# vvvwo/KSS-ICP

Measured on AMD Instinct MI355X. Metric: icp_iterations_per_sec, higher is better.
Workload: dtype f32; 1 GPU; C2: one 100000x100000 uniform-sphere pair per GPU, 50 fixed ICP iterations + fitness pass per step (exact NN + cov reduce + host 3x3 SVD), R_z(10deg), jitter 1e-3; n_src=100000, n_tgt=100000, pairs_per_gpu=1, nn_engine=cell list + brute-force fallback, nn_arithmetic=reference (no fma)

## Files before the change

### kss-icp_amd/csrc/kss_ctx.hpp

```cpp
#pragma once
#include <dlfcn.h>
#include <hip/hip_runtime.h>

#include <algorithm>
#include <atomic>
#include <chrono>
#include <cmath>
#include <cstdio>
#include <cstdlib>
#include <cstring>
#include <mutex>
#include <string>
#include <thread>
#include <vector>

#include "kss_internal.hpp"
#include "kss_host_pool.hpp"

using namespace kss;

struct DevBuf {
    void* p = nullptr;
    size_t cap = 0;
};
// ... 16 lines not shown
    double grid_stats[8] = {0, 0, 0, 0, 0, 0, 0, 0};
    double last_setup_ms = 0, last_loop_ms = 0;
    double t_launch_us = 0, t_wait_us = 0, t_host_us = 0;
    bool timing = false;
    bool tables_staged = false;
    int64_t stats_ns = -1, stats_nt = -1;

    DevBuf tgt4, src0, cur[2], keys, partials, sums, nn_work, red_work, pair_red, state, cs, scratch_a,
        scratch_b, scratch_c, stage_src, stage_tgt, stage_idx, stage_d2, stage_out, g_counts, g_slot, g_start, g_cursor,
        g_bsums, g_sorted, g_list, g_count, g_bbox, g_partials, g_start2, g_pairs, g_stamps, g_pos, g_nnst, res_pos, res_wc, res_perm, pack_seg, reg_s, reg_t, reg_p, reg_all, reg_f, reg_g, oct_pts, oct_cen, oct_a, oct_b, oct_tmp, pre_partials, pre_state, g_rowpair, g_gate;
    DevBuf p2l_idx, p2l_d2, p2l_perm, p2l_rows, p2l_nrm, p2l_n64;
    DevBuf trim_rows, trim_state;
    DevBuf rob_keys;
    DevBuf gicp_snrm;
    DevBuf pb_desc, pb_rowpair, pb_nrm;
    DevBuf pb_rscale;
    DevBuf pb_snrm, pb_gicp;
    DevBuf o2o_table, o2o_idx, o2o_d2;
    DevBuf recip_sorted, recip_box, recip_grids;
    std::vector<RecipPairDev> h_recip_grids;
    int64_t recip_total_cells = 0;
    void* h_gicp = nullptr; size_t h_gicp_cap = 0;
    void* h_gicp_dev = nullptr;
    const PairState* last_state_dev = nullptr;
    HostPool pool;
    std::vector<kss_vmap*> vmaps;
    std::vector<kss_ctx*> workers;
    std::vector<unsigned long long> last_stamps;
    int stamps_nblk = 0; unsigned long long stamps_seq = 0;
    std::vector<float> h_bbox;
    unsigned int* h_box = nullptr; unsigned int* h_box_dev = nullptr; size_t h_box_bytes = 0;
    unsigned box_tag = 0; int box_rows = 0;
    double evals_sum = 0.0, evals_launches = 0.0;
    void* h_sums = nullptr;  size_t h_sums_cap = 0;
    void* h_sums_dev = nullptr;
    void* h_p2l = nullptr; size_t h_p2l_cap = 0;
    void* h_p2l_dev = nullptr;
    unsigned long long* h_seq = nullptr;
    unsigned long long* h_seq_dev = nullptr;
    size_t h_seq_bytes = 0;
    struct Gated {
        int supported = -1;
        bool want_next = false;
        bool pending = false;
        bool chain = false;
        int steps_left = 0;
        int max_steps = 1;
        int slot = 0;
        unsigned long long seq = 0;
        int32_t stamp = 0;
        const void* d_in = nullptr; void* d_out = nullptr;
        bool fma = false, full = false, want_full = false; double max_d2 = 0.0;
    } gated;
    bool ws_dirty = false;
    bool defer_wait = false;
    PairState* h_xf = nullptr; PairState* h_xf_dev = nullptr;
    bool fit_last = false;
    bool nn_have = false;
    BarBuf gate_bar, res_gate, bar_state;
    int large_bar = -1;
    unsigned res_launches = 0;
    double res_passes = 0.0;
    int cand_cap = 0, cand_cap_pad = -1, cand_cap_fma = -1;
    int spec_judge = -1; double spec_threshold = 0.0; bool spec_ran = false, spec_cancelled = false;
    std::chrono::steady_clock::time_point res_backoff[2] = {};
    unsigned long long seq = 0;
    void* h_state = nullptr; size_t h_state_cap = 0;

    int prof = 0;
    unsigned prof_tick[KSS_K_COUNT] = {};
    struct EvPair { hipEvent_t a, b; };
    std::vector<EvPair> ev[KSS_K_COUNT];
    std::vector<EvPair> ev_pool;
    double prof_ms[KSS_K_COUNT] = {0};
    int64_t prof_n[KSS_K_COUNT] = {0};
};

static inline int set_err(kss_ctx* c, int code, const char* what, hipError_t e = hipSuccess) {
    if (c) {
        c->err = what;
        if (e != hipSuccess) { c->err += ": "; c->err += hipGetErrorString(e); }
    }
    return code;
}

#define HIPCHK(ctx, call)                                                        \
    do {                                                                         \
        hipError_t e_ = (call);                                                  \
        if (e_ != hipSuccess) return set_err((ctx), KSS_ERR_HIP, #call, e_);     \
    } while (0)

static inline int ensure(kss_ctx* c, DevBuf& b, size_t bytes) {
    if (bytes <= b.cap) return KSS_OK;
    if (b.p) {
        HIPCHK(c, hipStreamSynchronize(c->stream));
        HIPCHK(c, hipFree(b.p));
        b.p = nullptr; b.cap = 0;
    }
    size_t want = bytes + bytes / 8 + 256;
    hipError_t e = hipMalloc(&b.p, want);
    if (e != hipSuccess) { b.p = nullptr; return set_err(c, KSS_ERR_NOMEM, "hipMalloc", e); }
    b.cap = want;
    return KSS_OK;
}

static inline int ensure_zeroed(kss_ctx* c, DevBuf& b, size_t bytes) {
// ... 145 lines not shown
```

### kss-icp_amd/csrc/kss_engine.hip

```cpp
#pragma clang fp contract(off)

#include <emmintrin.h>
#include <limits>

#include "kss_ctx.hpp"
#include "kss_pair_device.hpp"

namespace kss {

static int restore_zero_at_rest(kss_ctx* c);

static int resident_rows_limit(kss_ctx* c) {
    if (c->cu_count <= 0) {
        hipDeviceProp_t prop;
        c->cu_count = hipGetDeviceProperties(&prop, c->device) == hipSuccess && prop.multiProcessorCount > 0 ? prop.multiProcessorCount : 1;
        (void)hipGetLastError();
    }
    return c->cu_count;
}

constexpr int PUB_PAIRS = 32;
static int ensure_pub(kss_ctx* c, int npairs = PUB_PAIRS);

struct PairGeom {
// ... 440 lines not shown
static void gated_cancel(kss_ctx* c);

static inline bool collect_pair(kss_ctx* c, int p, unsigned long long want) {
    const unsigned long long* sl = c->h_seq + (size_t)2 * NSUMS * p;
    double* out = (double*)c->h_sums + (size_t)NSUMS * p;
    if (!slots_collect(sl + 2 * (NSUMS - 1), 1, want, out + NSUMS - 1)) return false;
    return slots_collect(sl, NSUMS, want, out);
}

static int wait_pair(kss_ctx* c, int p, unsigned long long want) {
    for (long spin = 0; spin < 2000000; ++spin) {
        if (collect_pair(c, p, want)) return KSS_OK;
        __builtin_ia32_pause();
    }
    return KSS_ERR_HIP;
}

static int wait_seq(kss_ctx* c, int npairs = 1, unsigned long long want = 0, const int* active = nullptr, bool* not_published = nullptr) {
    if (!want) want = c->seq;
    bool slow = false;
    for (int p = npairs - 1; p >= 0; --p) {
        if (active && !active[p]) continue;
        if (!slow && wait_pair(c, p, want) == KSS_OK) continue;
        if (!slow) {
            gated_cancel(c);
            HIPCHK(c, hipStreamSynchronize(c->stream));
            slow = true;
        }
        if (!collect_pair(c, p, want)) {
            if (not_published) *not_published = true;
            return set_err(c, KSS_ERR_HIP, "kernel finished without publishing its result");
        }
    }
    return KSS_OK;
}

int ensure_pub_slots(kss_ctx* c) { return ensure_pub(c); }
int wait_slots(kss_ctx* c, int nslots, double* out) {
    const unsigned long long want = c->seq;
    for (long spin = 0; spin < 2000000; ++spin) {
        if (slots_collect(c->h_seq, nslots, want, out)) return KSS_OK;
        __builtin_ia32_pause();
    }
    HIPCHK(c, hipStreamSynchronize(c->stream));
    if (!slots_collect(c->h_seq, nslots, want, out)) return set_err(c, KSS_ERR_HIP, "kernel finished without publishing its result");
    return KSS_OK;
}

static bool gated_available(kss_ctx* c) {
    static const bool want = getenv("KSS_GATED") == nullptr || atoi(getenv("KSS_GATED")) != 0;
    if (!want || !c->own_stream || kss_live_contexts().load() != 1) return false;
    if (c->gated.supported < 0) {
        c->gated.supported = 0;
        if (bar_ensure(c, c->gate_bar, 256)) {
            c->gated.supported = 1;
            return true;
        }
        void *x = nullptr, *xd = nullptr;
        if (ensure(c, c->g_gate, 256) == KSS_OK && hipMemsetAsync(c->g_gate.p, 0, 256, c->stream) == hipSuccess &&
            hipHostMalloc(&x, 2 * sizeof(PairState), hipHostMallocMapped) == hipSuccess && hipHostGetDevicePointer(&xd, x, 0) == hipSuccess) {
            std::memset(x, 0, 2 * sizeof(PairState));
            c->h_xf = (PairState*)x; c->h_xf_dev = (PairState*)xd;
            c->gated.supported = 1;
        } else {
            (void)hipGetLastError();
            if (x) hipHostFree(x);
        }
    }
    return c->gated.supported == 1;
}

static void gated_release(kss_ctx* c, const PairState& st, int skip) {
    if (c->gate_bar.p) {
        unsigned words[16];
        std::memcpy(words, &st, sizeof st);
        words[14] = (unsigned)skip;
        static const long torn_at = getenv("KSS_TEST_TORN_GATE") ? atol(getenv("KSS_TEST_TORN_GATE")) : -1;
        static long released = 0;
        gate_record_store((unsigned*)c->gate_bar.p + 32 * c->gated.slot, words, (unsigned)c->gated.stamp, ++released == torn_at);
    } else {
        PairState* rec = &c->h_xf[c->gated.slot];
        for (int k = 0; k < 12; ++k) rec->m[k] = st.m[k];
        rec->active = st.active; rec->apply = st.apply; rec->pad[0] = skip;
        __atomic_store_n(&rec->pad[1], c->gated.stamp, __ATOMIC_RELEASE);
    }
    kss_ctx::Gated& G = c->gated;
    if (!skip && --G.steps_left > 0) {
        G.slot ^= 1;
        G.stamp += 1;
        G.seq += 1;
        const void* in = G.d_out; G.d_out = const_cast<void*>(G.d_in); G.d_in = in;
    } else {
        G.pending = false;
        G.steps_left = 0;
    }
}

static void gated_cancel(kss_ctx* c) {
    if (!c->gated.pending) return;
    PairState none;
    std::memset(&none, 0, sizeof none);
    gated_release(c, none, 1);
}

struct GatedGuard {
    kss_ctx* c;
    explicit GatedGuard(kss_ctx* c_) : c(c_) {}
    ~GatedGuard() { gated_cancel(c); c->gated.want_next = false; }
};

static float skin_setting() {
    static const float skin = getenv("KSS_SKIN") ? (float)atof(getenv("KSS_SKIN")) : 0.25f;
    return skin;
}
static int gate_polls_setting() {
    static const int gate_polls = getenv("KSS_GATE_POLLS") ? atoi(getenv("KSS_GATE_POLLS")) : (1 << 22);
    return gate_polls;
}

static PassArgs pass_args(kss_ctx* c, const IcpPlan& pl, const float4* d_in, float4* d_out, double max_d2,
                          int32_t* d_idx_out, float* d_d2_out) {
    PassArgs a;
    std::memset(&a, 0, sizeof a);
    a.src_in = d_in; a.src_out = d_out;
    a.cell_start = (const int32_t*)c->g_start.p + 1;
    a.sorted = (const float4*)c->g_sorted.p;
    a.tgt4 = (const float4*)c->tgt4.p;
    a.nn_win = (float4*)c->g_pos.p;
    a.nn_state = (float2*)c->g_nnst.p;
    a.skin = skin_setting();
    a.chain_len = 1;
    a.gate_polls = gate_polls_setting();
    a.chained = d_in != (const float4*)c->src0.p ? 1 : c->fit_last ? 2 : 0;
    a.src_last0 = (const float4*)c->cur[0].p; a.src_last1 = (const float4*)c->cur[1].p;
    a.keys = (unsigned long long*)c->keys.p;
    a.list = (int32_t*)c->g_list.p; a.list_count = (int32_t*)c->g_count.p;
    a.total_rows = pl.total_rows;
    a.use_prev = c->nn_have ? 1 : 0;
    a.max_d2 = max_d2;
    a.rows = (Granule*)c->partials.p;
    a.pub = c->h_seq_dev;
    a.idx_out = d_idx_out; a.d2_out = d_d2_out;
    {
        static const long torn_at = getenv("KSS_TEST_TORN_SLOT") ? atol(getenv("KSS_TEST_TORN_SLOT")) : -1;
        static long launches = 0;
        a.test_torn = torn_at > 0 && ++launches == torn_at ? 1 : 0;
    }
    if (pl.gridb) {
        a.pairs = (const GridPairDev*)c->g_pairs.p;
        a.row_pair = (const int32_t*)c->g_rowpair.p;
        a.defer_pairs = pl.npairs > resident_rows_limit(c) ? pl.npairs : 0;
    } else {
        a.pair0 = pl.gpairs[0];
    }
    return a;
}

struct GridPass {
    const IcpPlan& pl;
    bool fma, full;
    const float4* d_in; float4* d_out;
    double max_d2;
    int32_t* d_idx_out; float* d_d2_out;
    PassArgs a;
    int nblk;
    unsigned long long* stamps2 = nullptr;
    bool plain_args = false;
    unsigned long long want_seq = 0;
    bool via_gate = false;
};

static void grid_launch_plain(kss_ctx* c, GridPass& g) {
    ProfScope ps(c, KSS_K_GRID_NN);
    g.a.ps0 = ((const PairState*)c->h_state)[0];
    g.a.seq = ++c->seq;
    if (g.stamps2) g.a.stamps = g.stamps2 + (size_t)(g.a.seq & 1) * g.nblk * 16;
    launch_grid_pass(c->stream, g.fma, g.full, false, true, g.a);
    c->nn_have = true;
    g.want_seq = c->seq;
}

static void grid_release_or_launch(kss_ctx* c, GridPass& g) {
    kss_ctx::Gated& G = c->gated;
    if (G.pending && G.d_in == (const void*)g.d_in && G.d_out == (void*)g.d_out && G.fma == g.fma && G.full == g.full && G.max_d2 == g.max_d2 && g.plain_args) {
        g.want_seq = G.seq;
        c->seq = std::max(c->seq, G.seq);
        if (G.chain && c->prof > 0) c->prof_n[KSS_K_GRID_CHAIN_PASS] += 1;
        g.via_gate = true;
        static const long drop_at = getenv("KSS_TEST_DROP_GATE") ? atol(getenv("KSS_TEST_DROP_GATE")) : -1;
        static long releases = 0;
        if (++releases == drop_at) { G.pending = false; G.steps_left = 0; }
        else gated_release(c, ((const PairState*)c->h_state)[0], 0);
    } else {
        gated_cancel(c);
        grid_launch_plain(c, g);
    }
}

static void grid_enqueue_next(kss_ctx* c, const GridPass& g) {
    kss_ctx::Gated& G = c->gated;
    const bool next_sampled = c->prof == 1 || (c->prof > 1 && c->prof_tick[KSS_K_GRID_NN] % (unsigned)c->prof == 0);
    static const bool want_chain = getenv("KSS_CHAIN") == nullptr || atoi(getenv("KSS_CHAIN")) != 0;
    int len = 1;
    if (G.want_next && !G.pending && g.plain_args && gated_available(c) && want_chain && c->gate_bar.p &&
        (g.pl.total_rows <= resident_rows_limit(c) || g.pl.total_rows == 1))
        len = std::max(1, std::min(G.max_steps, 1 << 16));
    if (!(G.want_next && !G.pending && g.plain_args && gated_available(c) && (len > 1 || !next_sampled))) return;
    if (c->prof > 1 && len == 1) ++c->prof_tick[KSS_K_GRID_NN];
    float4* nxt_out = g.d_out == (float4*)c->cur[0].p ? (float4*)c->cur[1].p : (float4*)c->cur[0].p;
    G.slot ^= 1;
    G.stamp = (G.stamp + 1) & 0x7fffffff;
    if (G.stamp == 0 || G.stamp > 0x7fffffff - len - 1) G.stamp = 1;
    PassArgs n = pass_args(c, g.pl, g.d_out, nxt_out, g.max_d2, nullptr, nullptr);
    n.ps0 = ((const PairState*)c->h_state)[0];
    n.gate_seq = G.stamp;
    if (c->gate_bar.p) {
        n.state = nullptr;
        n.gate_dev = (unsigned int*)c->gate_bar.p;
        n.gate_slot = G.slot;
        n.chain_len = len;
        n.src_alt = g.d_out;
    } else {
        n.state = c->h_xf_dev + G.slot;
        n.gate_dev = (unsigned int*)c->g_gate.p;
    }
    n.seq = c->seq + 1;
    if (g.stamps2) n.stamps = g.stamps2 + (size_t)(n.seq & 1) * g.nblk * 16;
    if (len > 1) {
        ProfScope ps(c, KSS_K_GRID_CHAIN, true);
        launch_grid_pass(c->stream, g.fma, G.want_full, false, true, n);
    } else {
        launch_grid_pass(c->stream, g.fma, G.want_full, false, true, n);
    }
    G.chain = len > 1;
    G.pending = true; G.steps_left = len; G.seq = n.seq; G.d_in = g.d_out; G.d_out = nxt_out; G.fma = g.fma; G.full = G.want_full; G.max_d2 = g.max_d2;
    if (hipGetLastError() != hipSuccess) { gated_cancel(c); G.supported = 0; }
}

static int grid_wait(kss_ctx* c, GridPass& g) {
    bool not_published = false;
    const int rcw = wait_seq(c, 1, g.want_seq, nullptr, &not_published);
    if (rcw == KSS_OK || !g.via_gate || !not_published) return rcw;
    c->gated.pending = false; c->gated.steps_left = 0;
    c->err.clear();
    std::fprintf(stderr, "[kss] a waiting kernel was not answered in time and left; the pass is launched again\n");
    c->ws_dirty = true;
    KCHK(restore_zero_at_rest(c));
    grid_launch_plain(c, g);
    HIPCHK(c, hipGetLastError());
    return wait_seq(c, 1, g.want_seq);
}

static int grid_stamps_arm(kss_ctx* c, GridPass& g) {
    static const int stamps_mode = getenv("KSS_GRID_STAMPS") ? atoi(getenv("KSS_GRID_STAMPS")) : 0;
    if (stamps_mode == 1) {
        KCHK(ensure(c, c->g_stamps, (size_t)g.nblk * 16 * sizeof(unsigned long long)));
        HIPCHK(c, hipMemsetAsync(c->g_stamps.p, 0, (size_t)g.nblk * 16 * sizeof(unsigned long long), c->stream));
        g.a.stamps = (unsigned long long*)c->g_stamps.p;
    } else if (stamps_mode == 2) {
        KCHK(ensure(c, c->g_stamps, (size_t)g.nblk * 32 * sizeof(unsigned long long)));
        g.stamps2 = (unsigned long long*)c->g_stamps.p;
        c->stamps_nblk = g.nblk;
    }
    return KSS_OK;
}
static int grid_stamps_read(kss_ctx* c, const GridPass& g) {
    if (g.stamps2) { c->stamps_seq = g.want_seq; return KSS_OK; }
    if (!g.a.stamps) return KSS_OK;
    c->last_stamps.resize((size_t)g.nblk * 16);
    HIPCHK(c, hipMemcpy(c->last_stamps.data(), g.a.stamps, c->last_stamps.size() * sizeof(unsigned long long), hipMemcpyDeviceToHost));
    for (int b = 0; b < g.nblk; ++b) c->evals_sum += (double)c->last_stamps[(size_t)b * 16 + 10];
    c->evals_launches += 1.0;
    return KSS_OK;
}

static int grid_list_fallback(kss_ctx* c, const GridPass& g) {
    const IcpPlan& pl = g.pl;
    gated_cancel(c);
    c->gated.want_next = false;
    KCHK(stage_tables(c, pl));
    {
        PairState one;
        std::memset(&one, 0, sizeof one);
        one.active = 1;
        HIPCHK(c, hipMemcpy(c->state.p, &one, sizeof one, hipMemcpyHostToDevice));
    }
    if (getenv("KSS_LIST_CHECK")) {
        HIPCHK(c, hipStreamSynchronize(c->stream));
// ... 200 lines not shown
static int pair_ninfo(const PairMode& M) { return M.sim ? KSS_SIM_NINFO : M.mutual ? KSS_RECIP_NINFO : M.unique ? KSS_O2O_NINFO : KSS_TRIM_NINFO; }
static_assert(KSS_O2O_NINFO <= KSS_SIM_NINFO && KSS_RECIP_NINFO <= KSS_SIM_NINFO, "the loops' info arrays hold KSS_SIM_NINFO doubles");
static bool pair_host_step(const kss_icp_params& P, const PairMode& M, const double* s, double* info, PairTrack& t, bool trace) {
    if (M.sim) { info[4] = 0.0; info[5] = t.s_acc; }
    const double cnt = M.robust ? s[(M.plane ? P2L_NSUMS : NSUMS) - 1] : s[0];
    if ((int)cnt < P.min_correspondences) { t.state = KSS_STATE_NO_CORRESPONDENCES; return false; }
    float ck[16];
    const float* crit = t.tk;
    double scale_dev2 = 0.0;
    if (M.symm) {
        if (!rigid_from_symm_sums(s, t.tk)) { t.state = KSS_STATE_DEGENERATE; return false; }
    } else if (M.plane) {
        if (!rigid_from_p2l_sums(s, t.tk)) { t.state = KSS_STATE_DEGENERATE; return false; }
    } else if (M.sim) {
        double sk;
        if (!sim_from_sums(s, M.scale_min / t.s_acc, M.scale_max / t.s_acc, t.tk, &sk, ck)) { t.state = KSS_STATE_DEGENERATE; return false; }
        t.s_acc = std::fmin(std::fmax(t.s_acc * sk, M.scale_min), M.scale_max);
        info[4] = sk; info[5] = t.s_acc;
        scale_dev2 = (sk - 1.0) * (sk - 1.0);
        crit = ck;
    } else {
        rigid_from_sums(s, t.tk);
    }
    mat4_mul(t.tk, t.fin, t.fin);
    ++t.iters;
    const double mse = (M.plane ? s[28] : s[16]) / s[0];
    t.last_mse = mse;
    if (trace) trace_row(P, s, M.plane ? P2L_NSUMS : NSUMS, t.tk, M.trimmed || M.robust ? M.trace_info : nullptr, info, pair_ninfo(M));
    const bool done = t.cv.has_converged(t.iters, crit, mse, scale_dev2);
    t.state = t.cv.state;
    if (done) t.converged = 1;
    return !done;
}
static int fitness_corr_out(kss_ctx* c, const kss_icp_params& P, const int32_t* d_idx, const float* d_d2, size_t n0) {
    if (P.fitness_idx) HIPCHK(c, hipMemcpyAsync(P.fitness_idx, d_idx, n0 * sizeof(int32_t), hipMemcpyDeviceToHost, c->stream));
    if (P.fitness_d2) HIPCHK(c, hipMemcpyAsync(P.fitness_d2, d_d2, n0 * sizeof(float), hipMemcpyDeviceToHost, c->stream));
    HIPCHK(c, hipStreamSynchronize(c->stream));
    return KSS_OK;
}
static int fitness_pass(kss_ctx* c, const IcpPlan& pl, const kss_icp_params& P, const PairTrack* tr, bool claim_last,
                        PairState* bar, int32_t* d_idx, float* d_d2, kss_icp_result* results) {
    const int np = pl.npairs;
    PairState* hs = (PairState*)c->h_state;
    const bool claim = claim_last && (pl.grid || pl.gridb);
    for (int p = 0; p < np; ++p) {
        set_state(hs[p], tr[p].fin, 1, 1);
        if (claim && tr[p].iters >= 1 && tr[p].state != KSS_STATE_NO_CORRESPONDENCES && tr[p].state != KSS_STATE_DEGENERATE)
            hs[p].pad[0] = 1 + ((tr[p].iters - 1) & 1);
        mirror_state(bar, p, hs[p]);
    }
    c->fit_last = claim;
    struct FitGuard { kss_ctx* c; ~FitGuard() { c->fit_last = false; } } fit_guard{c};
    c->gated.want_next = false;
    KCHK(nn_pass(c, pl, P.nn_fma != 0, (const float4*)c->src0.p, (float4*)c->cur[0].p, P.max_corr_dist * P.max_corr_dist, d_idx, d_d2, true));
    const double* hsum = (const double*)c->h_sums;
    if (P.allreduce) {
        double v[2] = {hsum[17], (double)pl.g[0].ns};
        if (P.allreduce(P.allreduce_user, v, 2) != 0) return set_err(c, KSS_ERR_RCCL, "icp: the allreduce callback failed");
        results[0].fitness = v[0] / v[1];
    } else {
        for (int p = 0; p < np; ++p) results[p].fitness = hsum[(size_t)p * NSUMS + 17] / (double)pl.g[p].ns;
    }
    if (d_idx) KCHK(fitness_corr_out(c, P, d_idx, d_d2, (size_t)pl.g[0].ns));
    return KSS_OK;
}

static bool resident_capacities(const IcpPlan& pl, int* ntc_out, int* tabc_out) {
    int64_t max_nt = 0;
    for (int p = 0; p < pl.npairs; ++p) {
        if (pl.g[p].ns > (int64_t)RES_SMAX * RES_THREADS || pl.g[p].nt > 65534) return false;
        max_nt = std::max(max_nt, pl.g[p].nt);
    }
    const int ntc = (int)((max_nt + 3 + 63) / 64 * 64);
    const int64_t avail = ((int64_t)RES_LDS_MAX - (int64_t)resident_lds_bytes(ntc, 0)) / 2 / 8 * 8;
    if (avail < 16) return false;
    int64_t want = 16;
    for (int p = 0; p < pl.npairs; ++p) {
        const GridParams& gp = pl.gpairs[p].gp;
        const int64_t rows = (int64_t)gp.gy * gp.gz;
        int xs = 0;
        while (xs <= 8 && rows * (((gp.gx + (1 << xs) - 1) >> xs) + 1) > avail) ++xs;
        if (xs > 8) return false;
        want = std::max(want, rows * (((gp.gx + (1 << xs) - 1) >> xs) + 1));
    }
    *ntc_out = ntc;
    *tabc_out = (int)((want + 7) / 8 * 8);
    return true;
}

static std::atomic<int> g_cand_in_flight[64];
struct CandReservation {
    int dev = -1, n = 0;
    bool take(int device, int want, int cap) {
        if (device < 0 || device >= 64 || n != 0) return false;
        const int before = g_cand_in_flight[device].fetch_add(want);
        if (before + want > cap) { g_cand_in_flight[device].fetch_sub(want); return false; }
        dev = device; n = want;
        return true;
    }
    ~CandReservation() { if (n > 0) g_cand_in_flight[dev].fetch_sub(n); }
};

struct ResLaunch {
    bool launched = false;
    unsigned long long seq0 = 0; unsigned stamp0 = 0;
    int32_t* idx_out = nullptr; float* d2_out = nullptr;
// ... 332 lines not shown

static int switch_engine_on_fallback(kss_ctx* c, const IcpPlan*& plan, IcpPlan& brute_plan, const kss_icp_params& P,
                                     const std::vector<int>& was_active) {
    const int np = plan->npairs;
    const double* hsum = (const double*)c->h_sums;
    double fallback = 0.0, act = 0.0;
    for (int p = 0; p < np; ++p)
        if (was_active[p]) { fallback += hsum[(size_t)p * NSUMS + NSUMS - 1]; act += (double)plan->g[p].ns; }
    if (!(fallback > 0.10 * act) || getenv("KSS_GRID_NOSWITCH")) return KSS_OK;
    std::vector<int64_t> ns(np), nt(np);
    for (int p = 0; p < np; ++p) { ns[p] = plan->g[p].ns; nt[p] = plan->g[p].nt; }
    KCHK(build_plan(c, ns.data(), nt.data(), np, false, P.nn_sources_per_thread, P.nn_target_splits, KSS_NN_BRUTE, brute_plan));
    brute_plan.src_in_cell_order = true;
    KCHK(stage_plan(c, brute_plan));
    plan = &brute_plan;
    return KSS_OK;
}

static int icp_loop(kss_ctx* c, const IcpPlan& pl_in, const kss_icp_params& P, kss_icp_result* results) {
    if (pl_in.gridb) {
        bool handled = false;
        KCHK(resident_loop(c, pl_in, P, results, &handled));
        if (handled) return KSS_OK;
    }
    if (!pl_in.grid && !pl_in.gridb && pl_in.shared_target) {
        bool handled = false;
        KCHK(resident_loop(c, pl_in, P, results, &handled, true));
        if (handled) return KSS_OK;
    }
    if (c->spec_judge >= 0) return KSS_OK;
    const IcpPlan* plan = &pl_in;
    IcpPlan brute_plan;
    const int np = pl_in.npairs;
    std::vector<PairTrack> tr((size_t)np, PairTrack(P));
    std::vector<int> active(np, 1), solved(np, 0), was_active;
    const PairMode plain;
    const bool full = P.trace_sums != nullptr;
    PairState* hs = (PairState*)c->h_state;
    PairState* bar = pl_in.gridb ? (PairState*)bar_ensure(c, c->bar_state, (size_t)np * sizeof(PairState)) : nullptr;
    float I[16];
    mat4_identity(I);
    for (int p = 0; p < np; ++p) {
        set_state(hs[p], I, 1, 0);
        mirror_state(bar, p, hs[p]);
    }
    const double max_d2 = P.max_corr_dist * P.max_corr_dist;
    const double* hsum = (const double*)c->h_sums;
    if (P.trace_n) *P.trace_n = 0;
    int n_active = P.max_iterations > 0 ? np : 0;
    if (P.max_iterations <= 0)
        for (int p = 0; p < np; ++p) { active[p] = 0; }
    int it = 0;
    GatedGuard gated_guard(c);

    auto solve_pairs = [&](int p0, int p1, unsigned long long pass_seq, bool poll_first, int* n_finished) -> int {
        std::atomic<int> finished{0}, stuck{0};
        bool poll = poll_first;
        std::fill(solved.begin() + p0, solved.begin() + p1, 0);
        auto solve = [&](int pb, int pe) {
            int fin_here = 0;
            for (int p = pb; p < pe; ++p) {
                if (!active[p] || solved[p]) continue;
                if (poll && wait_pair(c, p, pass_seq) != KSS_OK) { stuck.fetch_add(1); continue; }
                PairTrack& t = tr[p];
                const bool goes_on = pair_host_step(P, plain, hsum + (size_t)p * NSUMS, nullptr, t, p == 0);
                solved[p] = 1;
                if (goes_on) {
                    set_state(hs[p], t.tk, 1, 1);
                } else {
                    active[p] = 0; ++fin_here;
                    if (t.state == KSS_STATE_NO_CORRESPONDENCES) set_state(hs[p], I, 0, 0);
                    else set_state(hs[p], t.tk, 0, 1);
                }
                mirror_state(bar, p, hs[p]);
            }
            finished.fetch_add(fin_here, std::memory_order_relaxed);
        };
        const int n = p1 - p0;
        if (n >= 64) {
            std::atomic<int> next{0};
            constexpr int kBlock = 64;
            c->pool.parallel_for(n, [&](int, int) {
                for (;;) {
                    const int pb = p0 + next.fetch_add(1) * kBlock;
                    if (pb >= p1) break;
                    solve(pb, std::min(p1, pb + kBlock));
                }
            });
        } else {
            solve(p0, p1);
        }
        if (stuck.load() > 0) {
            HIPCHK(c, hipStreamSynchronize(c->stream));
            for (int p = p0; p < p1; ++p) {
                if (!active[p] || solved[p]) continue;
                if (!collect_pair(c, p, pass_seq)) return set_err(c, KSS_ERR_HIP, "kernel finished without publishing its result");
            }
            poll = false;
            solve(p0, p1);
        }
        *n_finished = finished.load(std::memory_order_relaxed);
        return KSS_OK;
    };

    while (n_active > 0) {
        const float4* d_in = it == 0 ? (const float4*)c->src0.p : (const float4*)c->cur[(it - 1) & 1].p;
        float4* d_out = (float4*)c->cur[it & 1].p;
        c->gated.want_next = plan->grid && !P.allreduce && it + 1 < P.max_iterations;
        c->gated.want_full = full;
        c->gated.max_steps = P.max_iterations - (it + 1);
        c->defer_wait = plan->gridb;
        const auto tb0 = c->timing ? std::chrono::steady_clock::now() : std::chrono::steady_clock::time_point();
        const int rc_pass = nn_pass(c, *plan, P.nn_fma != 0, d_in, d_out, max_d2, nullptr, nullptr, full, active.data());
        const bool deferred = c->defer_wait;
        c->defer_wait = false;
        const auto tb1 = c->timing ? std::chrono::steady_clock::now() : std::chrono::steady_clock::time_point();
        KCHK(rc_pass);
        const unsigned long long pass_seq = c->seq;
        if (P.allreduce && P.allreduce(P.allreduce_user, (double*)c->h_sums, NSUMS) != 0)
            return set_err(c, KSS_ERR_RCCL, "icp: the allreduce callback failed");
        if (plan->gridb) was_active = active;
        int fin_now = 0;
        KCHK(solve_pairs(0, np, pass_seq, deferred, &fin_now));
        if (c->timing && deferred) {
            const auto tb2 = std::chrono::steady_clock::now();
            c->t_launch_us += std::chrono::duration<double, std::micro>(tb1 - tb0).count();
            c->t_wait_us += std::chrono::duration<double, std::micro>(tb2 - tb1).count();
        }
        if (plan->gridb) KCHK(switch_engine_on_fallback(c, plan, brute_plan, P, was_active));
        n_active -= fin_now;
        ++it;
    }
    for (int p = 0; p < np; ++p) fill_result(results[p], tr[p].fin, tr[p].iters, tr[p].converged, tr[p].state, tr[p].last_mse, 0.0, p);
    if (!P.compute_fitness) return KSS_OK;
    int32_t* d_idx = nullptr;
    float* d_d2 = nullptr;
    if (P.fitness_idx || P.fitness_d2) {
        KCHK(ensure(c, c->stage_idx, (size_t)plan->total_src * sizeof(int32_t)));
        KCHK(ensure(c, c->stage_d2, (size_t)plan->total_src * sizeof(float)));
        d_idx = (int32_t*)c->stage_idx.p; d_d2 = (float*)c->stage_d2.p;
    }
    return fitness_pass(c, *plan, P, tr.data(), plan == &pl_in, bar, d_idx, d_d2, results);
}

static int restore_zero_at_rest(kss_ctx* c) {
    if (!c->ws_dirty) return KSS_OK;
    HIPCHK(c, hipStreamSynchronize(c->stream));
    for (DevBuf* b : {&c->g_count, &c->g_counts})
        if (b->p) HIPCHK(c, hipMemsetAsync(b->p, 0, b->cap, c->stream));
    c->ws_dirty = false;
    return KSS_OK;
}
struct DirtyGuard {
    kss_ctx* c; bool ok = false;
    explicit DirtyGuard(kss_ctx* c_) : c(c_) {}
    ~DirtyGuard() { if (!ok) c->ws_dirty = true; }
};

int icp_run_dev(kss_ctx* c, const void* d_src, const int64_t* src_off, const void* d_tgt, const int64_t* tgt_off,
                int npairs, bool shared_target, int dtype, const kss_icp_params* p, kss_icp_result* results) {
    if (!c || !d_src || !d_tgt || !src_off || !tgt_off || !p || !results || npairs <= 0) return set_err(c, KSS_ERR_ARG, "icp: bad argument");
    if (p->allreduce && npairs != 1) return set_err(c, KSS_ERR_ARG, "icp: the source-row split (allreduce) is for a single pair");
    HIPCHK(c, hipSetDevice(c->device));
    std::vector<int64_t> ns(npairs), nt(npairs);
    for (int i = 0; i < npairs; ++i) {
        ns[i] = src_off[i + 1] - src_off[i];
        nt[i] = shared_target ? tgt_off[1] - tgt_off[0] : tgt_off[i + 1] - tgt_off[i];
    }
    IcpPlan pl;
    const auto t0 = std::chrono::steady_clock::now();
    KCHK(restore_zero_at_rest(c));
    DirtyGuard guard(c);
    c->timing = getenv("KSS_TIMING") != nullptr;
    auto lap = [&](const char* what, std::chrono::steady_clock::time_point& from) {
        if (!c->timing) return;
        const auto now = std::chrono::steady_clock::now();
        std::fprintf(stderr, "[kss]   %s %.1f us\n", what, std::chrono::duration<double, std::micro>(now - from).count());
        from = now;
    };
    auto ts = t0;
    KCHK(build_plan(c, ns.data(), nt.data(), npairs, shared_target, p->nn_sources_per_thread, p->nn_target_splits, p->nn_mode, pl));
    lap("plan", ts);
    KCHK(stage_plan(c, pl));
    lap("stage", ts);
    KCHK(pack_clouds(c, pl, d_src, src_off, d_tgt, tgt_off, dtype));
    lap("pack (enqueue)", ts);
    KCHK(grid_setup(c, pl));
    KCHK(grid_setup_batch(c, pl));
    lap("cell lists (bbox sync + enqueue)", ts);
    if (c->timing) HIPCHK(c, hipStreamSynchronize(c->stream));
    lap("drain", ts);
    const auto t1 = std::chrono::steady_clock::now();
    c->t_launch_us = c->t_wait_us = 0;
    const int rc = icp_loop(c, pl, *p, results);
// ... 630 lines not shown
```

### kss-icp_amd/csrc/kss_grid.hip

```cpp
#pragma clang fp contract(off)

#include <hip/hip_runtime.h>

#include <cstring>

#include <rocprim/rocprim.hpp>

#include <cstdlib>

#include "kss_internal.hpp"
#include "kss_device.hpp"

namespace kss {

__global__ __launch_bounds__(256) void grid_count2_kernel(const float4* __restrict__ tgt, int nt, int nbt, const float4* __restrict__ src, int ns,
                                                          GridParams gp, int32_t* __restrict__ counts, int32_t* __restrict__ slot) {
    const bool is_src = (int)blockIdx.x >= nbt;
    const int i = ((int)blockIdx.x - (is_src ? nbt : 0)) * 256 + (int)threadIdx.x;
    if (i >= (is_src ? ns : nt)) return;
    const float4 p = is_src ? src[i] : tgt[i];
    const int cx = cell_coord(p.x, gp.ox, gp.inv_h, gp.gx), cy = cell_coord(p.y, gp.oy, gp.inv_h, gp.gy),
              cz = cell_coord(p.z, gp.oz, gp.inv_h, gp.gz);
    slot[(is_src ? nt : 0) + i] = atomicAdd(&counts[(is_src ? gp.gx * gp.gy * gp.gz : 0) + (cz * gp.gy + cy) * gp.gx + cx], 1);
}
// ... 612 lines not shown
        }
    }
#undef KSS_STAMP
}

#ifndef KSS_SINGLE_WAVES
#define KSS_SINGLE_WAVES 1
#endif
template <bool FMA, bool FULL, bool SEARCH, bool CHAIN, bool FIRST = false>
__global__ __launch_bounds__(PASS_BS, KSS_SINGLE_WAVES) void grid_pass_kernel(const PassArgs a) {
    static_assert(!CHAIN || SEARCH, "chained launches: search passes");
    static_assert(!FIRST || (SEARCH && !CHAIN), "the first pass: a plain search launch");
#define KSS_STAMP(k) do { if (a.stamps && threadIdx.x == 0) a.stamps[(size_t)blockIdx.x * 16 + (k)] = __builtin_amdgcn_s_memrealtime(); } while (0)
    KSS_STAMP(0);
    constexpr int BS = PASS_BS;
    const int per_xcd = (int)gridDim.x / 8;
    const int w = ((int)blockIdx.x % 8) * per_xcd + (int)blockIdx.x / 8;
    if (w >= a.total_rows) return;
    const GridPairDev pr = a.pair0;
    PairState ps = a.ps0;
    const GridParams& gp = pr.gp;
    const int32_t* __restrict__ cs = a.cell_start + pr.cell_base;
    const float4* __restrict__ sorted = a.sorted;
    constexpr int WQ = FIRST ? BS : 256;
    __shared__ int2 rowq[9][WQ];
    __shared__ double shw[BS / 64][NSUMS];
    __shared__ int s_last;
    __shared__ int sh_ps[16];
    __shared__ int s_nwalk;
    __shared__ unsigned s_ent[7][BS];
    __shared__ unsigned short s_wl[BS];
    enum { WK_X, WK_Y, WK_Z, WK_IDX, WK_D2, WK_R, WK_POS, WK_FL = WK_POS, WK_COLS };
    static_assert(sizeof(PairState) == 64, "the gated launch reads the transform record as 16 dwords");
    double (*shf)[NSUMS] = reinterpret_cast<double (*)[NSUMS]>(&rowq[0][0]);
    static_assert(sizeof(double) * PASS_FG * NSUMS <= sizeof(int2) * 9 * WQ, "shf must fit inside rowq");

    const int local = (w - pr.row_base) * BS + (int)threadIdx.x;
    const bool valid = local < pr.src_n;
    const int i = pr.src_base + local;
    const int lane = threadIdx.x & 63, wave = threadIdx.x >> 6;
    bool have = false, fell_back = false;
    float qx = 0.f, qy = 0.f, qz = 0.f, d2 = 0.f;
    float4 win = make_float4(0.f, 0.f, 0.f, 0.f);
    float4 p = make_float4(0.f, 0.f, 0.f, 0.f), prevp = make_float4(0.f, 0.f, 0.f, __uint_as_float(~0u));
    float2 st = make_float2(0.f, 0.f);
    if (valid) {
        p = SEARCH ? a.src_in[i] : a.src_out[i];
        if (!SEARCH || a.use_prev) { prevp = a.nn_win[i]; st = a.nn_state[i]; }
    }
    for (int step = 0;; ++step) {
    const bool last_step = !CHAIN || step + 1 >= a.chain_len;
    const unsigned long long seq_k = a.seq + (unsigned long long)step;
    const int gate_k = a.gate_seq != 0 ? a.gate_seq + step : 0;
    unsigned int* const gate_ptr = a.gate_dev + 32 * ((a.gate_slot + step) & 1);
    float4* const src_out_k = (step & 1) ? a.src_alt : a.src_out;
    const bool last_known = a.chained == 2 && ps.pad[0] > 0;
    const bool chained_k = step > 0 || a.chained == 1 || last_known;
    const bool has_prev = __float_as_uint(prevp.w) != ~0u;
    if constexpr (SEARCH) {
        __syncthreads();
        if (threadIdx.x == 0) s_nwalk = 0;
        __syncthreads();
    }
    KSS_STAMP(13);
    if constexpr (SEARCH) {
        if (gate_k != 0) {
            typedef unsigned int u32x4 __attribute__((ext_vector_type(4)));
            if (a.state && w == 0 && threadIdx.x < 16) {
                const int* w32 = reinterpret_cast<const int*>(a.state);
                int v = 0, n = 0;
                bool ok = true;
                for (;;) {
                    v = __hip_atomic_load(w32 + threadIdx.x, __ATOMIC_RELAXED, __HIP_MEMORY_SCOPE_SYSTEM);
                    if (__shfl(v, 15, 64) == gate_k) break;
                    __builtin_amdgcn_s_sleep(1);
                    if (++n > a.gate_polls / 2) { ok = false; break; }
                }
                if (ok) {
                    const int g = threadIdx.x;
                    const int w0 = __shfl(v, min(3 * g, 15), 64), w1 = __shfl(v, min(3 * g + 1, 15), 64), w2 = __shfl(v, min(3 * g + 2, 15), 64);
                    if (g < 5) {
                        u32x4 o;
                        o.x = (unsigned)w0; o.y = (unsigned)w1; o.z = (unsigned)w2; o.w = (unsigned)gate_k + kss_mix3(o.x, o.y, o.z);
                        unsigned int* dst = gate_ptr + 4 * g;
                        asm volatile("global_store_dwordx4 %0, %1, off sc1" ::"v"(dst), "v"(o) : "memory");
                    }
                }
            }
            if (threadIdx.x < 8) {
                const unsigned int* src = gate_ptr + 4 * min((int)threadIdx.x, 4);
                u32x4 v;
                int n = 0;
                bool ok = true;
                for (;;) {
                    asm volatile("global_load_dwordx4 %0, %1, off sc0 sc1\n\ts_waitcnt vmcnt(0)" : "=&v"(v) : "v"(src) : "memory");
                    if (__builtin_amdgcn_ballot_w64(v.w - kss_mix3(v.x, v.y, v.z) == (unsigned)gate_k) == 0xffull) break;
                    __builtin_amdgcn_s_sleep(1);
                    if (++n > a.gate_polls) { ok = false; break; }
                }
                if (threadIdx.x < 5) { sh_ps[3 * threadIdx.x] = (int)v.x; sh_ps[3 * threadIdx.x + 1] = (int)v.y; sh_ps[3 * threadIdx.x + 2] = (int)v.z; }
                if (threadIdx.x == 0) { sh_ps[15] = gate_k; s_last = ok ? 1 : 0; }
            }
            __syncthreads();
            if (!s_last) return;
            int* d32 = reinterpret_cast<int*>(&ps);
#pragma unroll
            for (int k = 0; k < 16; ++k) d32[k] = sh_ps[k];
            if (ps.pad[0] != 0) return;
            __syncthreads();
            KSS_STAMP(9);
        }
    }
    unsigned long long key = ~0ull;
    float pold_x = p.x, pold_y = p.y, pold_z = p.z;
    if (SEARCH && last_known && valid) {
        const float4 pl = (ps.pad[0] == 1 ? a.src_last0 : a.src_last1)[i];
        pold_x = pl.x; pold_y = pl.y; pold_z = pl.z;
    }
    if (valid) {
        if constexpr (SEARCH) {
            if (ps.apply) {
                const float x = p.x, y = p.y, z = p.z;
                p.x = ((ps.m[0] * x + ps.m[1] * y) + ps.m[2] * z) + ps.m[3];
                p.y = ((ps.m[4] * x + ps.m[5] * y) + ps.m[6] * z) + ps.m[7];
                p.z = ((ps.m[8] * x + ps.m[9] * y) + ps.m[10] * z) + ps.m[11];
            }
            src_out_k[i] = p;
        }
        qx = p.x; qy = p.y; qz = p.z;
        const bool qok = (qx - qx) == 0.f && (qy - qy) == 0.f && (qz - qz) == 0.f;
        if constexpr (!SEARCH) {
            if (has_prev) {
                win = prevp;
                key = point_key<FMA>(win, qx, qy, qz);
            } else if (qok) {
                key = a.keys[i];
                if (key != ~0ull) win = a.tgt4[pr.tgt_base + (int)(unsigned)(key & 0xffffffffull)];
            }
            have = key != ~0ull;
        }
    }
    if constexpr (SEARCH) {
        bool walker = false;
        float acc_keep = 0.f;
        {
            const bool qok = valid && (qx - qx) == 0.f && (qy - qy) == 0.f && (qz - qz) == 0.f;
            const SkipOut so = skip_test<FMA>(qok, qx, qy, qz, pold_x, pold_y, pold_z, prevp, st, chained_k, a.skin, gp.h);
            walker = so.walker;
            key = so.key;
            acc_keep = so.acc;
            unsigned fl = 0u;
            if (qok && !walker) {
                fl = 1u;
                a.nn_state[i] = make_float2(st.x, so.acc);
            } else if (valid && !qok) {
                a.nn_win[i] = make_float4(0.f, 0.f, 0.f, __uint_as_float(~0u));
                a.nn_state[i] = make_float2(0.f, 0.f);
            }
            const float4 c4 = walker ? make_float4(qx, qy, qz, 0.f) : prevp;
            s_ent[WK_X][threadIdx.x] = __float_as_uint(c4.x); s_ent[WK_Y][threadIdx.x] = __float_as_uint(c4.y); s_ent[WK_Z][threadIdx.x] = __float_as_uint(c4.z);
            s_ent[WK_IDX][threadIdx.x] = (unsigned)key; s_ent[WK_D2][threadIdx.x] = (unsigned)(key >> 32);
            s_ent[WK_POS][threadIdx.x] = walker ? (unsigned)so.kpos : fl;
            s_ent[WK_R][threadIdx.x] = __float_as_uint(so.rho);
        }
        const unsigned long long wm = __builtin_amdgcn_ballot_w64(walker);
        if (wm != 0ull) {
            int base = 0;
            if (lane == 0) base = atomicAdd(&s_nwalk, (int)__builtin_popcountll(wm));
            base = __builtin_amdgcn_readfirstlane(base);
// ... 574 lines not shown
```

### kss-icp_amd/csrc/kss_internal.hpp

```cpp
#pragma once
#include <hip/hip_runtime.h>

#include <algorithm>
#include <cfloat>
#include <cmath>
#include <cstdint>
#include <functional>
#include <string>
#include <vector>

#include "../../include/kssicp.h"
#include "kss_handover.hpp"
#include "kss_host_math.hpp"

namespace kss {

struct alignas(16) PairState {
    float m[12];
    int32_t active;
    int32_t apply;
    int32_t pad[2];
};

struct alignas(16) NNWork {
// ... 28 lines not shown
    float h, inv_h;
    float eps;
    int32_t gx, gy, gz;
    int32_t rcap;
};

struct alignas(16) GridPairDev {
    GridParams gp;
    int32_t cell_base;
    int32_t tgt_base, tgt_n;
    int32_t src_base, src_n;
    int32_t tgt_pad;
    int32_t row_base, n_rows;
    int32_t sorted_base;
};

struct PackSeg {
    int64_t in_off;
    int64_t out_base;
    int64_t n;
};

struct alignas(16) Granule { unsigned long long bits, seq; };

struct PassArgs {
    const float4* src_in; float4* src_out;
    const int32_t* cell_start;
    const float4* sorted;
    const float4* tgt4;
    float4* nn_win;
    float2* nn_state;
    int32_t chained;
    const float4* src_last0; const float4* src_last1;
    float skin;
    unsigned long long* keys;
    int32_t* list; int32_t* list_count;
    const GridPairDev* pairs;
    const int32_t* row_pair;
    const PairState* state;
    GridPairDev pair0; PairState ps0;
    int32_t total_rows, use_prev;
    int32_t gate_polls;
    int32_t chain_len, gate_slot;
    float4* src_alt;
    int32_t gate_seq;
    int32_t defer_pairs;
    unsigned int* gate_dev;
    double max_d2;
    Granule* rows;
    unsigned long long* pub; unsigned long long seq;
    int32_t* idx_out; float* d2_out;
    unsigned long long* stamps;
    int32_t test_torn;
};

constexpr int RES_THREADS = 1024;
constexpr int RES_SMAX = 10;
constexpr int RES_NQ = 640;
constexpr int RES_QW = 4;
constexpr int RES_G = 4;
constexpr int RES_LDS_MAX = 160 * 1024 - 256;
struct ResArgs {
    const GridPairDev* pairs;
    const int32_t* cell_start;
    const float4* sorted;
    const float4* src0;
    unsigned int* gate;
    unsigned long long* pub;
    unsigned long long seq0;
    unsigned int stamp0;
    double max_d2;
    float skin;
    int32_t gate_polls, max_passes, full_always;
    int32_t ntc, tabc;
    int32_t* idx_out; float* d2_out;
    unsigned long long* exit_flags;
    unsigned int exit_tag;
    const int32_t* perm;
    int32_t first_pass, split_at;
    float4* st_pos; unsigned int* st_wc;
    unsigned long long* stamps;
};
size_t resident_lds_bytes(int ntc, int tabc);
int launch_resident(hipStream_t st, bool fma, int npairs, const ResArgs& a, std::string& err);

struct OctBox {
    double min[3], max[3];
    double res;
    int32_t depth;
};

constexpr int NN_TILE = 256;
constexpr int NN_SUB = 32;
constexpr int NN_THREADS = 256;

inline void oct_first_point(OctBox& b, const float* p) {
    const float minValue = FLT_EPSILON;
    for (int k = 0; k < 3; ++k) { b.min[k] = p[k] - b.res / 2; b.max[k] = p[k] + b.res / 2; }
    unsigned maxv = 2;
    for (int k = 0; k < 3; ++k) maxv = std::max(maxv, (unsigned)std::ceil((b.max[k] - b.min[k] - minValue) / b.res));
    b.depth = (int)std::ceil(std::log2((double)maxv) - minValue);
    const double side = (double)(1u << b.depth) * b.res;
    for (int k = 0; k < 3; ++k) {
        const double over = (side - (b.max[k] - b.min[k])) / 2.0;
        if (over > minValue) { b.min[k] -= over; b.max[k] += over; }
    }
// ... 306 lines not shown
```

Before: 82100 iterations/s.

## Pre-enqueue gated fitness pass behind final ICP chain to hide launch latency

After: 82800 iterations/s, median of 4. No clear change (+0.8%).

```diff
diff --git a/kss-icp_amd/csrc/kss_ctx.hpp b/kss-icp_amd/csrc/kss_ctx.hpp
--- a/kss-icp_amd/csrc/kss_ctx.hpp
+++ b/kss-icp_amd/csrc/kss_ctx.hpp
@@ -92,6 +92,17 @@
         const void* d_in = nullptr; void* d_out = nullptr;
         bool fma = false, full = false, want_full = false; double max_d2 = 0.0;
     } gated;
+    struct FitGated {
+        bool want = false;
+        int last_buf = 0;
+        int32_t* idx_out = nullptr; float* d2_out = nullptr;
+        bool pending = false;
+        const void* plan = nullptr;
+        unsigned long long seq = 0;
+        int32_t stamp = 0;
+        int32_t last_stamp = 0;
+        bool fma = false; double max_d2 = 0.0;
+    } fit;
     bool ws_dirty = false;
     bool defer_wait = false;
     PairState* h_xf = nullptr; PairState* h_xf_dev = nullptr;
diff --git a/kss-icp_amd/csrc/kss_engine.hip b/kss-icp_amd/csrc/kss_engine.hip
--- a/kss-icp_amd/csrc/kss_engine.hip
+++ b/kss-icp_amd/csrc/kss_engine.hip
@@ -516,7 +516,7 @@
     if (!want || !c->own_stream || kss_live_contexts().load() != 1) return false;
     if (c->gated.supported < 0) {
         c->gated.supported = 0;
-        if (bar_ensure(c, c->gate_bar, 256)) {
+        if (bar_ensure(c, c->gate_bar, 384)) {
             c->gated.supported = 1;
             return true;
         }
@@ -560,18 +560,33 @@
     }
 }
 
+static void fit_release(kss_ctx* c, const PairState& st, int skip) {
+    unsigned words[16];
+    std::memcpy(words, &st, sizeof st);
+    words[14] = (unsigned)skip;
+    gate_record_store((unsigned*)c->gate_bar.p + 32 * 2, words, (unsigned)c->fit.stamp, false);
+    c->fit.pending = false;
+}
+
 static void gated_cancel(kss_ctx* c) {
-    if (!c->gated.pending) return;
+    if (!c->gated.pending && !c->fit.pending) return;
     PairState none;
     std::memset(&none, 0, sizeof none);
-    gated_release(c, none, 1);
+    if (c->gated.pending) gated_release(c, none, 1);
+    if (c->fit.pending) fit_release(c, none, 1);
 }
 
 struct GatedGuard {
     kss_ctx* c;
     explicit GatedGuard(kss_ctx* c_) : c(c_) {}
-    ~GatedGuard() { gated_cancel(c); c->gated.want_next = false; }
+    ~GatedGuard() { gated_cancel(c); c->gated.want_next = false; c->fit.want = false; }
 };
+
+static bool gate_answer_dropped() {
+    static const long drop_at = getenv("KSS_TEST_DROP_GATE") ? atol(getenv("KSS_TEST_DROP_GATE")) : -1;
+    static long releases = 0;
+    return ++releases == drop_at;
+}
 
 static float skin_setting() {
     static const float skin = getenv("KSS_SKIN") ? (float)atof(getenv("KSS_SKIN")) : 0.25f;
@@ -646,15 +661,26 @@
 
 static void grid_release_or_launch(kss_ctx* c, GridPass& g) {
     kss_ctx::Gated& G = c->gated;
+    kss_ctx::FitGated& F = c->fit;
+    const PairState& hs0 = ((const PairState*)c->h_state)[0];
+    if (F.pending && !G.pending && c->fit_last && g.full && g.d_in == (const float4*)c->src0.p && g.d_out == (float4*)c->cur[0].p && F.plan == (const void*)&g.pl &&
+        F.fma == g.fma && F.max_d2 == g.max_d2 && F.idx_out == g.d_idx_out && F.d2_out == g.d_d2_out && !g.a.stamps && hs0.pad[0] == F.last_buf &&
+        F.seq == c->seq + 1) {
+        g.want_seq = F.seq;
+        c->seq = F.seq;
+        g.via_gate = true;
+        if (c->prof > 1) ++c->prof_tick[KSS_K_GRID_NN];
+        if (gate_answer_dropped()) F.pending = false;
+        else fit_release(c, hs0, 0);
+        return;
+    }
     if (G.pending && G.d_in == (const void*)g.d_in && G.d_out == (void*)g.d_out && G.fma == g.fma && G.full == g.full && G.max_d2 == g.max_d2 && g.plain_args) {
         g.want_seq = G.seq;
         c->seq = std::max(c->seq, G.seq);
         if (G.chain && c->prof > 0) c->prof_n[KSS_K_GRID_CHAIN_PASS] += 1;
         g.via_gate = true;
-        static const long drop_at = getenv("KSS_TEST_DROP_GATE") ? atol(getenv("KSS_TEST_DROP_GATE")) : -1;
-        static long releases = 0;
-        if (++releases == drop_at) { G.pending = false; G.steps_left = 0; }
-        else gated_release(c, ((const PairState*)c->h_state)[0], 0);
+        if (gate_answer_dropped()) { G.pending = false; G.steps_left = 0; }
+        else gated_release(c, hs0, 0);
     } else {
         gated_cancel(c);
         grid_launch_plain(c, g);
@@ -673,8 +699,9 @@
     if (c->prof > 1 && len == 1) ++c->prof_tick[KSS_K_GRID_NN];
     float4* nxt_out = g.d_out == (float4*)c->cur[0].p ? (float4*)c->cur[1].p : (float4*)c->cur[0].p;
     G.slot ^= 1;
-    G.stamp = (G.stamp + 1) & 0x7fffffff;
-    if (G.stamp == 0 || G.stamp > 0x7fffffff - len - 1) G.stamp = 1;
+    kss_ctx::FitGated& F = c->fit;
+    G.stamp = (std::max(G.stamp, F.last_stamp) + 1) & 0x7fffffff;
+    if (G.stamp == 0 || G.stamp > 0x7fffffff - len - 2) { G.stamp = 1; F.last_stamp = 0; }
     PassArgs n = pass_args(c, g.pl, g.d_out, nxt_out, g.max_d2, nullptr, nullptr);
     n.ps0 = ((const PairState*)c->h_state)[0];
     n.gate_seq = G.stamp;
@@ -698,6 +725,20 @@
     }
     G.chain = len > 1;
     G.pending = true; G.steps_left = len; G.seq = n.seq; G.d_in = g.d_out; G.d_out = nxt_out; G.fma = g.fma; G.full = G.want_full; G.max_d2 = g.max_d2;
+    static const bool want_fit = getenv("KSS_FIT_GATED") == nullptr || atoi(getenv("KSS_FIT_GATED")) != 0;
+    const bool fit_sampled = c->prof == 1 || (c->prof > 1 && c->prof_tick[KSS_K_GRID_NN] % (unsigned)c->prof == 0);
+    if (want_fit && F.want && !F.pending && len == G.max_steps && c->gate_bar.p && !g.stamps2 && !fit_sampled &&
+        (g.pl.total_rows <= resident_rows_limit(c) || g.pl.total_rows == 1)) {
+        PassArgs f = n;
+        f.src_in = (const float4*)c->src0.p; f.src_out = (float4*)c->cur[0].p; f.src_alt = nullptr;
+        f.chained = 2; f.last_buf = F.last_buf;
+        f.chain_len = 1; f.gate_slot = 2; f.gate_seq = G.stamp + len;
+        f.seq = n.seq + (unsigned long long)len;
+        f.idx_out = F.idx_out; f.d2_out = F.d2_out;
+        f.test_torn = 0;
+        launch_grid_pass(c->stream, g.fma, true, false, true, f);
+        F.pending = true; F.plan = &g.pl; F.seq = f.seq; F.stamp = F.last_stamp = f.gate_seq; F.fma = g.fma; F.max_d2 = g.max_d2;
+    }
     if (hipGetLastError() != hipSuccess) { gated_cancel(c); G.supported = 0; }
 }
 
@@ -1004,6 +1045,7 @@
     c->fit_last = claim;
     struct FitGuard { kss_ctx* c; ~FitGuard() { c->fit_last = false; } } fit_guard{c};
     c->gated.want_next = false;
+    if (c->fit.pending && !(claim && np == 1 && tr[0].iters == P.max_iterations && d_idx == c->fit.idx_out && d_d2 == c->fit.d2_out)) gated_cancel(c);
     KCHK(nn_pass(c, pl, P.nn_fma != 0, (const float4*)c->src0.p, (float4*)c->cur[0].p, P.max_corr_dist * P.max_corr_dist, d_idx, d_d2, true));
     const double* hsum = (const double*)c->h_sums;
     if (P.allreduce) {
@@ -1442,6 +1484,21 @@
         for (int p = 0; p < np; ++p) { active[p] = 0; }
     int it = 0;
     GatedGuard gated_guard(c);
+    int32_t* d_idx = nullptr;
+    float* d_d2 = nullptr;
+    auto corr_buffers = [&]() -> int {
+        if (!P.compute_fitness || !(P.fitness_idx || P.fitness_d2) || d_idx) return KSS_OK;
+        KCHK(ensure(c, c->stage_idx, (size_t)plan->total_src * sizeof(int32_t)));
+        KCHK(ensure(c, c->stage_d2, (size_t)plan->total_src * sizeof(float)));
+        d_idx = (int32_t*)c->stage_idx.p; d_d2 = (float*)c->stage_d2.p;
+        return KSS_OK;
+    };
+    if (plan->grid && np == 1 && P.compute_fitness && !P.allreduce && P.max_iterations > 0) {
+        KCHK(corr_buffers());
+        c->fit.want = true;
+        c->fit.last_buf = 1 + ((P.max_iterations - 1) & 1);
+        c->fit.idx_out = d_idx; c->fit.d2_out = d_d2;
+    }
 
     auto solve_pairs = [&](int p0, int p1, unsigned long long pass_seq, bool poll_first, int* n_finished) -> int {
         std::atomic<int> finished{0}, stuck{0};
@@ -1523,13 +1580,7 @@
     }
     for (int p = 0; p < np; ++p) fill_result(results[p], tr[p].fin, tr[p].iters, tr[p].converged, tr[p].state, tr[p].last_mse, 0.0, p);
     if (!P.compute_fitness) return KSS_OK;
-    int32_t* d_idx = nullptr;
-    float* d_d2 = nullptr;
-    if (P.fitness_idx || P.fitness_d2) {
-        KCHK(ensure(c, c->stage_idx, (size_t)plan->total_src * sizeof(int32_t)));
-        KCHK(ensure(c, c->stage_d2, (size_t)plan->total_src * sizeof(float)));
-        d_idx = (int32_t*)c->stage_idx.p; d_d2 = (float*)c->stage_d2.p;
-    }
+    KCHK(corr_buffers());
     return fitness_pass(c, *plan, P, tr.data(), plan == &pl_in, bar, d_idx, d_d2, results);
 }
 
diff --git a/kss-icp_amd/csrc/kss_grid.hip b/kss-icp_amd/csrc/kss_grid.hip
--- a/kss-icp_amd/csrc/kss_grid.hip
+++ b/kss-icp_amd/csrc/kss_grid.hip
@@ -688,9 +688,10 @@
     const bool last_step = !CHAIN || step + 1 >= a.chain_len;
     const unsigned long long seq_k = a.seq + (unsigned long long)step;
     const int gate_k = a.gate_seq != 0 ? a.gate_seq + step : 0;
-    unsigned int* const gate_ptr = a.gate_dev + 32 * ((a.gate_slot + step) & 1);
+    unsigned int* const gate_ptr = a.gate_dev + 32 * (!CHAIN && a.gate_slot == 2 ? 2 : (a.gate_slot + step) & 1);
     float4* const src_out_k = (step & 1) ? a.src_alt : a.src_out;
-    const bool last_known = a.chained == 2 && ps.pad[0] > 0;
+    const int claim = !CHAIN && a.chained == 2 && a.gate_seq != 0 ? a.last_buf : ps.pad[0];
+    const bool last_known = a.chained == 2 && claim > 0;
     const bool chained_k = step > 0 || a.chained == 1 || last_known;
     const bool has_prev = __float_as_uint(prevp.w) != ~0u;
     if constexpr (SEARCH) {
@@ -750,7 +751,7 @@
     unsigned long long key = ~0ull;
     float pold_x = p.x, pold_y = p.y, pold_z = p.z;
     if (SEARCH && last_known && valid) {
-        const float4 pl = (ps.pad[0] == 1 ? a.src_last0 : a.src_last1)[i];
+        const float4 pl = (claim == 1 ? a.src_last0 : a.src_last1)[i];
         pold_x = pl.x; pold_y = pl.y; pold_z = pl.z;
     }
     if (valid) {
diff --git a/kss-icp_amd/csrc/kss_internal.hpp b/kss-icp_amd/csrc/kss_internal.hpp
--- a/kss-icp_amd/csrc/kss_internal.hpp
+++ b/kss-icp_amd/csrc/kss_internal.hpp
@@ -104,6 +104,7 @@
     int32_t* idx_out; float* d2_out;
     unsigned long long* stamps;
     int32_t test_torn;
+    int32_t last_buf;
 };
 
 constexpr int RES_THREADS = 1024;
```
